# cmusatyalab/mega-nerf

Measured on NVIDIA B200. Metric: ray-samples/sec (MLP+composite), higher is better.
Workload: dtype f16 operands / f32 accumulate

## Files before the change

include/mn_b200.h:

```cpp
#ifndef MN_B200_H
#define MN_B200_H

#include <stddef.h>
#include <stdint.h>

#ifdef __cplusplus
extern "C" {
#endif

#define MN_ABI_VERSION 1

enum {
    MN_OK = 0,
    MN_ERR_INVALID = 1,
    MN_ERR_CUDA = 2,
    MN_ERR_SHAPE = 3,
    MN_ERR_SPHERE = 4,
    MN_ERR_WORKSPACE = 5,
    MN_ERR_UNSUPPORTED = 6
};

enum {
    MN_PREC_FP32 = 0,
    MN_PREC_TC_F16 = 1,
// ... 111 lines not shown


int mn_composite_backward(mn_ctx* ctx, const float* raw_d, const float* z_d, int S, const float* raw2_d,
                          const float* z2_d, int S2, const float* last_delta_d, int64_t N, int flip,
                          const float* grad_rgb_d, const float* grad_lambda_d, float* grad_raw_d, float* grad_raw2_d,
                          void* stream);
int mn_sh_to_rgb_backward(mn_ctx* ctx, int deg, const float* coef_d, int64_t coef_stride, const float* dirs_d,
                          int64_t dir_stride, int dir_div, int64_t B, int apply_sigmoid, const float* grad_out_d,
                          float* grad_coef_d, void* stream);

size_t mn_model_tape_bytes(const mn_model* m, int64_t B);
int mn_model_forward_train(mn_ctx* ctx, mn_model* m, const mn_rows* rows, int64_t B, int use_coarse,
                           const float* sigma_noise_d, float* out_d, void* tape_d, size_t tape_bytes, void* workspace_d,
                           size_t workspace_bytes, void* stream);
#define MN_PARAM_OFFSETS 44
size_t mn_model_backward_workspace_bytes(const mn_model* m, int64_t B);
int64_t mn_model_grad_floats(const mn_model* m);
int mn_model_param_offsets(const mn_model* m, int64_t* out, int n);
int mn_model_backward(mn_ctx* ctx, mn_model* m, int64_t B, int use_coarse, const float* grad_out_d, const void* tape_d,
                      size_t tape_bytes, float* param_grads_d, void* workspace_d, size_t workspace_bytes, void* stream);

int mn_model_train_tc_supported(const mn_model* m);
size_t mn_model_tape_bytes_tc(const mn_model* m, int64_t B);
int mn_model_forward_train_tc(mn_ctx* ctx, mn_model* m, const mn_rows* rows, int64_t B, int use_coarse,
                              const float* sigma_noise_d, float* out_d, void* tape_d, size_t tape_bytes, void* workspace_d,
                              size_t workspace_bytes, void* stream);
size_t mn_model_backward_workspace_bytes_tc(const mn_model* m, int64_t B);
int mn_model_backward_tc(mn_ctx* ctx, mn_model* m, int64_t B, int use_coarse, const float* grad_out_d, const void* tape_d,
                         size_t tape_bytes, float* param_grads_d, void* workspace_d, size_t workspace_bytes, void* stream);

int mn_debug_tp_program(const mn_model_desc* desc, unsigned int* table_out, int cap_entries, int* info8);
int mn_debug_read_trace(unsigned long long* out, unsigned int* counts, int reset);
int mn_debug_read_clock(unsigned long long* out4);

#ifdef __cplusplus
}
#endif
#endif
```

mega_nerf_b200/_cabi.py:

```python
from __future__ import annotations

import ctypes as C
import os
import threading
from typing import Dict, Optional

import torch

_HERE = os.path.dirname(os.path.abspath(__file__))
LIB_PATH = os.path.join(_HERE, 'libmn_b200.so')

MN_OK, MN_ERR_INVALID, MN_ERR_CUDA, MN_ERR_SHAPE, MN_ERR_SPHERE, MN_ERR_WORKSPACE, MN_ERR_UNSUPPORTED = range(7)
PREC_FP32, PREC_TC_F16, PREC_TC_F16X3 = 0, 1, 2
PRECISIONS = {'fp32': PREC_FP32, 'tc_f16': PREC_TC_F16, 'tc_f16x3': PREC_TC_F16X3}

MN_MAX_LAYERS = 16


class ModelDesc(C.Structure):
    _fields_ = [('kind', C.c_int), ('n_sub', C.c_int),
                ('pos_xyz_dim', C.c_int), ('pos_dir_dim', C.c_int), ('layers', C.c_int), ('layer_dim', C.c_int),
                ('appearance_dim', C.c_int), ('affine_appearance', C.c_int), ('appearance_count', C.c_int),
                ('rgb_dim', C.c_int), ('xyz_dim', C.c_int), ('shifted_softplus', C.c_int),
                ('n_skip', C.c_int), ('skip_layers', C.c_int * 8),
                ('boundary_margin', C.c_float), ('xyz_real', C.c_int), ('cluster_dim_start', C.c_int)]


class NerfWeights(C.Structure):
    _fields_ = [('xyz_w', C.c_void_p * MN_MAX_LAYERS), ('xyz_b', C.c_void_p * MN_MAX_LAYERS),
                ('sigma_w', C.c_void_p), ('sigma_b', C.c_void_p), ('final_w', C.c_void_p), ('final_b', C.c_void_p),
                ('dir_a_w', C.c_void_p), ('dir_a_b', C.c_void_p), ('rgb_w', C.c_void_p), ('rgb_b', C.c_void_p),
                ('embedding_a', C.c_void_p), ('affine_w', C.c_void_p), ('affine_b', C.c_void_p)]


class Rows(C.Structure):
    _fields_ = [('mode', C.c_int), ('x_d', C.c_void_p), ('cols', C.c_int), ('dirs_d', C.c_void_p),
                ('dir_stride', C.c_int64), ('idx_d', C.c_void_p), ('samples_per_ray', C.c_int)]


_P, _I, _L, _F, _Z = C.c_void_p, C.c_int, C.c_int64, C.c_float, C.c_size_t
SIGNATURES = {
    'mn_abi_version': (_I, []),
    'mn_create': (_I, [C.POINTER(_P), _I]),
    'mn_destroy': (None, [_P]),
    'mn_last_error': (C.c_char_p, [_P]),
    'mn_check_status': (_I, [_P, _P]),
    'mn_launch_count': (C.c_longlong, [_P]),
    'mn_profile_enable': (_I, [_P, _I]),
    'mn_profile_read': (_I, [_P, C.POINTER(C.c_double), C.POINTER(C.c_longlong)]),
    'mn_ray_directions': (_I, [_P, _I, _I, _F, _F, _F, _F, _I, _P, _P]),
    'mn_rays': (_I, [_P, _P, _I, _P, _I, _L, _F, _F, _I, _F, _F, _P, _P]),
    'mn_rays_pairs': (_I, [_P, _P, _L, _P, _I, _P, _P, _L, _F, _F, _I, _F, _F, _P, _P]),
    'mn_debug_tp_program': (_I, [_P, _P, _I, _P]),
    'mn_debug_read_trace': (_I, [_P, _P, _I]),
    'mn_debug_read_clock': (_I, [_P]),
    'mn_sample_coarse': (_I, [_P, _P, _P, _P, _P, _F, _L, _I, _P, _P, _P]),
    'mn_stratify': (_I, [_P, _P, _L, _P, _F, _L, _I, _P, _P]),
    'mn_points_from_z': (_I, [_P, _P, _P, _L, _I, _P, _P]),
    'mn_sample_pdf': (_I, [_P, _P, _P, _L, _P, _P, _L, _L, _I, _I, _P, _P, _P, _P]),
    'mn_sort_cat': (_I, [_P, _P, _I, _P, _I, _L, _I, _P, _P]),
    'mn_composite': (_I, [_P, _P, _P, _P, _I, _P, _P, _P, _I, _P, _L, _I, _P, _P, _P, _P, _P, _P]),
    'mn_intersect_sphere': (_I, [_P, _P, _P, _P, _L, _P, _P]),
    'mn_points_outside': (_I, [_P, _P, _P, _P, _P, _P, _L, _I, _I, _I, _P, _P, _P]),
    'mn_sh_to_rgb': (_I, [_P, _I, _P, _L, _P, _L, _I, _L, _I, _P, _P]),
    'mn_embed': (_I, [_P, _P, _L, _I, _I, _P, _P]),
    'mn_model_create': (_I, [_P, C.POINTER(ModelDesc), C.POINTER(_P)]),
    'mn_model_destroy': (None, [_P]),
    'mn_model_set_centroids': (_I, [_P, _P, _P]),
    'mn_model_set_weights': (_I, [_P, _I, C.POINTER(NerfWeights), _P]),
    'mn_model_set_max_multiplicity': (_I, [_P, _I]),
    'mn_model_workspace_bytes': (_Z, [_P, _L, _I]),
    'mn_model_forward': (_I, [_P, _P, C.POINTER(Rows), _L, _I, _I, _P, _I, _P, _P, _Z, _P]),
    'mn_model_route': (_I, [_P, _P, C.POINTER(Rows), _L, _P, _P, _P]),
    'mn_model_last_stats': (_I, [_P, _P, C.POINTER(_L), C.POINTER(_L), _P]),
    'mn_render_rays_workspace_bytes': (_Z, [_P, _L, _I, _I, _I, _I, _I]),
    'mn_render_rays': (_I, [_P, _P, _P, _P, _L, _P, _I, _P, _I, _I, _I, _I, _P, _P, _P, _P, _P, _Z, _P]),
    'mn_peer_gather_store': (_I, [_P, _P, _P, _L, _L, C.POINTER(C.c_void_p), _I, _P]),
    'mn_cluster_min_dist_ratios': (_I, [_P, _P, _L, _P, _I, _P, _I, _I, _F, _P, _P, _P]),
    'mn_composite_backward': (_I, [_P, _P, _P, _I, _P, _P, _I, _P, _L, _I, _P, _P, _P, _P, _P]),
    'mn_sh_to_rgb_backward': (_I, [_P, _I, _P, _L, _P, _L, _I, _L, _I, _P, _P, _P]),
    'mn_model_tape_bytes': (_Z, [_P, _L]),
    'mn_model_forward_train': (_I, [_P, _P, C.POINTER(Rows), _L, _I, _P, _P, _P, _Z, _P, _Z, _P]),
    'mn_model_backward_workspace_bytes': (_Z, [_P, _L]),
    'mn_model_grad_floats': (_L, [_P]),
    'mn_model_param_offsets': (_I, [_P, C.POINTER(_L), _I]),
    'mn_model_backward': (_I, [_P, _P, _L, _I, _P, _P, _Z, _P, _P, _Z, _P]),
    'mn_model_train_tc_supported': (_I, [_P]),
    'mn_model_tape_bytes_tc': (_Z, [_P, _L]),
# ... 74 lines not shown
```

mega_nerf_b200/csrc/mn_mlp_tc.cu:

```cuda
#include <cuda_fp16.h>

#include <cstdlib>
#include <cstring>
#include <type_traits>
#include <vector>

#include "mn_model.cuh"

namespace {

constexpr int kTileM = 128;

__device__ unsigned long long g_trace[4 * 4096];
__device__ unsigned int g_trace_n[2];
__device__ __forceinline__ void trace_ev(int on, int who, int ev, int sl, int gi) {
    if (!(on & 1) || blockIdx.x != 0) return;
    const unsigned int i = atomicAdd(&g_trace_n[who], 1u);
    if (i < 2048) {
        unsigned long long t;
        asm volatile("mov.u64 %0, %%globaltimer;" : "=l"(t));
        g_trace[(who * 2048 + i) * 2 + 0] = ((unsigned long long)ev << 32) | ((unsigned long long)sl << 16) | (unsigned long long)gi;
        g_trace[(who * 2048 + i) * 2 + 1] = t;
    }
}
__device__ unsigned long long g_clk[4];
__device__ __forceinline__ void clk_stamp(int on, int which) {
    if (!(on & 1) || blockIdx.x != 0 || threadIdx.x != 0) return;
    unsigned long long t;
    asm volatile("mov.u64 %0, %%globaltimer;" : "=l"(t));
    g_clk[2 * which] = (unsigned long long)clock64();
    g_clk[2 * which + 1] = t;
}
constexpr int kMaxStages = 4;
__host__ __device__ constexpr int ring_slab_cols(bool split) { return split ? 32 : 64; }
__host__ __device__ constexpr int ring_stage_bytes(bool split) { return ring_slab_cols(split) * 256 * 2; }
constexpr int kMaxGemm = 16;
constexpr int kThreads = 576;
constexpr int kEpiWarps = 16;
constexpr int kWarpProd = 16;
constexpr int kWarpMma = 17;
constexpr int kPPThreads = kThreads;

enum { SRC_H = 0, SRC_XPE = 1, SRC_XAUX = 2 };
enum { EPI_RELU = 0, EPI_RELU_SIGMA = 1, EPI_LINEAR = 2, EPI_RGB = 3,
       EPI_D_LINEAR = 4, EPI_D_MASK = 5, EPI_D_MASK_SIGMA = 6 };
enum { PP_INFER = 0, PP_TRAIN_FWD = 1, PP_DGRAD = 2 };

struct TcGemm {
    int n;
    int nseg;
    int src[2];
    int k[2];
    int w_off;
    int bias_off;
    int epi;
};

struct TcPlan {
    int n_gemm, n_trunk;
    TcGemm g[kMaxGemm];
    int kpe, kaux;
    int plane_bytes;
    int f32_floats;
    int sigma_w_off;
// ... 505 lines not shown
        "add.u64 b1, %3, %4;\n\tadd.u64 b2, b1, %4;\n\tadd.u64 b3, b2, %4;\n\t"
        "@e  tcgen05.mma.cta_group::1.kind::f16 [%0], %1, %3, %5, p;\n\t"
        "@q1 tcgen05.mma.cta_group::1.kind::f16 [%0], a1, b1, %5, 1;\n\t"
        "@q2 tcgen05.mma.cta_group::1.kind::f16 [%0], a2, b2, %5, 1;\n\t"
        "@q3 tcgen05.mma.cta_group::1.kind::f16 [%0], a3, b3, %5, 1;\n\t"
        "@e  tcgen05.commit.cta_group::1.mbarrier::arrive::one.shared::cluster.b64 [%8];\n\t}"
        ::"r"(d_tmem), "l"(ad), "l"(a_step), "l"(bd), "l"(b_step), "r"(idesc), "r"(accum), "r"(nk), "r"(empty_bar)
        : "memory");
}


struct TcArgs {
    MlpArgs m;
    TcPlan plan;
    const unsigned char* wpack;
    const __half* ximg;
    int64_t x_plane_halves;
    int split;
    int desc_swap;
    int64_t n_tiles_cap;
    unsigned char* tape_act;
    float* tape_f32;
    unsigned char* tape_dz;
    float* tape_gf32;
    const float* grad_out;
    float* emb_sum;
    const float* scale;
    int64_t act_tile_bytes;
    int layers;
    const unsigned char* tpack;
    size_t tp_sub_bytes;
    const uint4* tp_prog;
    int tp_n[4];
};

struct SmemLayout {
    int ring, h, xa, f32, sigp, bars, total, stages;
};

constexpr int kSmemMax = 227 * 1024;

__host__ __device__ inline SmemLayout smem_layout(const TcPlan& p, bool split) {
    SmemLayout s;
    const int kx = p.kpe > p.kaux ? p.kpe : p.kaux;
    const int fixed = p.L * kTileM * 2 * (split ? 2 : 1) + kx * kTileM * 2 + ((p.f32_floats * 4 + 15) / 16) * 16 + 2048 + 256;
    int st = (kSmemMax - fixed) / ring_stage_bytes(split);
    if (st > kMaxStages) st = kMaxStages;
    s.stages = st;
    s.ring = 0;
    s.h = s.ring + st * ring_stage_bytes(split);
    s.xa = s.h + p.L * kTileM * 2 * (split ? 2 : 1);
    s.f32 = s.xa + kx * kTileM * 2;
    s.sigp = s.f32 + ((p.f32_floats * 4 + 15) / 16) * 16;
    s.bars = s.sigp + 2048;
    s.total = s.bars + 256;
    return s;
}

template <bool kSplit>
__global__ void __launch_bounds__(kThreads, 1) tc_mlp_kernel(const TcArgs A) {
    constexpr int kSlabCols = ring_slab_cols(kSplit);
    constexpr int kStageBytes = ring_stage_bytes(kSplit);
    extern __shared__ __align__(1024) unsigned char smem[];
    const TcPlan& P = A.plan;
    const SmemLayout SL = smem_layout(P, kSplit);
    const int kStages = SL.stages;
// ... 799 lines not shown
    }
    if ((rc = pack(P.g[gi++], Pk + m->lay.rgb_w, nd.rgb_dim, nd.rgb_in, 0, 0, Pk + m->lay.rgb_b, nd.rgb_dim))) return rc;
    mn_pack_push(ctx, PackOp{Pk + m->lay.sigma_w, f32 + P.sigma_w_off, nullptr, (long long)nd.L, PK_TC_F32, {nd.L, 0, 0, 0, 0, 0, 0}});
    mn_pack_push(ctx, PackOp{Pk + m->lay.sigma_b, f32 + P.sigma_w_off + nd.L, nullptr, 4, PK_TC_F32, {1, 0, 0, 0, 0, 0, 0}});
    m->tc_ready = 1;

    TcPlan D;
    m->train_tc_ok = 0;
    if (!wide && build_dgrad_plan(nd, &D)) {
        if (!m->tc_dgrad) {
            MN_CUDA(ctx, cudaMalloc(&m->tc_dgrad, (size_t)D.sub_bytes * m->d.n_sub));
            MN_CUDA(ctx, cudaMemsetAsync(m->tc_dgrad, 0, (size_t)D.sub_bytes * m->d.n_sub, st));
            m->tc_dgrad_sub_bytes = (size_t)D.sub_bytes;
        }
        unsigned char* db = (unsigned char*)m->tc_dgrad + (size_t)sub * D.sub_bytes;
        const float* Q = m->packed_bwd + (size_t)sub * m->blay.total;
        auto packd = [&](const TcGemm& g, const float* wd, int ld) -> int {
            mn_pack_push(ctx, PackOp{wd, db + g.w_off, nullptr, (long long)g.n * g.k[0], PK_DGRAD, {ld, g.n, g.k[0], 0, 0, 0, 0}});
            return MN_OK;
        };
        int di = 0;
        if ((rc = packd(D.g[di++], Q + m->blay.dira_f, nd.L))) return rc;
        if ((rc = packd(D.g[di++], Q + m->blay.final_w, nd.L))) return rc;
        for (int l = nd.layers - 1; l >= 1; --l)
            if ((rc = packd(D.g[di++], Q + m->blay.w[l], nd.L))) return rc;
        float* df32 = reinterpret_cast<float*>(db + D.f32_off);
        mn_pack_push(ctx, PackOp{Pk + m->lay.sigma_w, df32, nullptr, (long long)nd.L, PK_TC_F32, {nd.L, 0, 0, 0, 0, 0, 0}});
        mn_pack_push(ctx, PackOp{Pk + m->lay.rgb_w, df32 + nd.L, nullptr, (long long)3 * (nd.L / 2), PK_RGBW, {nd.L / 2, 3, 0, 0, 0, 0, 0}});
        m->train_tc_ok = 1;
    }
    return MN_OK;
}

int mn_mlp_tc_launch(mn_ctx* ctx, mn_model* m, const MlpArgs& a, int64_t n_tiles128, int precision, void* ws, size_t ws_bytes,
                     cudaStream_t st) {
    TcArgs A{};
    if (!build_plan(a.nd, &A.plan) || !m->tc_ready)
        return mn_fail(ctx, MN_ERR_UNSUPPORTED,
                       "tensor-core MLP path covers layer_dim 64..256 (multiple of 64) or 512 and rgb_dim <= 32; "
                       "use precision 'fp32' for this model");
    if (a.nd.L > 256 && precision == MN_PREC_TC_F16X3)
        return mn_fail(ctx, MN_ERR_UNSUPPORTED,
                       "precision 'tc_f16x3' covers layer_dim <= 256; use 'tc_f16' or 'fp32' for the 512-wide network");
    if (n_tiles128 <= 0) return MN_OK;
    TcPlan& P = A.plan;
    const int split = precision == MN_PREC_TC_F16X3 ? 1 : 0;
    P.sub_bytes = (int)m->tc_sub_bytes;
    A.m = a;
    A.wpack = (const unsigned char*)m->tc_packed;
    A.split = split;
    static int desc_swap = -1;
    if (desc_swap < 0) {
        const char* e = getenv("MN_TC_TRACE");
        desc_swap = e ? atoi(e) : 0;
    }
    A.desc_swap = desc_swap;
    A.n_tiles_cap = n_tiles128;
    const size_t need = mn_mlp_tc_workspace(m, n_tiles128, precision);
    if (ws_bytes < need || !ws) return mn_fail(ctx, MN_ERR_WORKSPACE, "mn_mlp_tc_launch: workspace too small");
    uintptr_t wp = ((uintptr_t)ws + 1023) / 1024 * 1024;
    __half* ximg = reinterpret_cast<__half*>(wp);
    A.ximg = ximg;
    A.x_plane_halves = (int64_t)n_tiles128 * (P.kpe + P.kaux) * kTileM;

    static int use_pp = -1;
    if (use_pp < 0) {
// ... 41 lines not shown
            const unsigned ncl = (unsigned)(groups < ctx->sm_count / 2 ? groups : ctx->sm_count / 2);
            cudaLaunchConfig_t cfg{};
            cfg.gridDim = dim3(2 * ncl);
            cfg.blockDim = dim3(kThreads);
            cfg.dynamicSmemBytes = (size_t)WL.total;
            cfg.stream = st;
            cudaLaunchAttribute at[1];
            at[0].id = cudaLaunchAttributeClusterDimension;
            at[0].val.clusterDim.x = 2;
            at[0].val.clusterDim.y = 1;
            at[0].val.clusterDim.z = 1;
            cfg.attrs = at;
            cfg.numAttrs = 1;
            MN_CUDA(ctx, cudaLaunchKernelEx(&cfg, tc_mlp_wide_kernel<2>, A));
        } else {
            MN_CUDA(ctx, cudaFuncSetAttribute(tc_mlp_wide_kernel<1>, cudaFuncAttributeMaxDynamicSharedMemorySize, WL.total));
            const unsigned grid_w = (unsigned)(n_tiles128 < ctx->sm_count ? n_tiles128 : ctx->sm_count);
            tc_mlp_wide_kernel<1><<<grid_w, kThreads, WL.total, st>>>(A);
        }
        mn_prof_end(ctx, st);
        MN_LAUNCH_CHECK(ctx);
        return MN_OK;
    }
    const SmemLayout SL = smem_layout(P, split != 0);
    const int total = SL.total;
    if (total > kSmemMax || SL.stages < 2) return mn_fail(ctx, MN_ERR_UNSUPPORTED, "tensor-core MLP: shared-memory budget exceeded");
    const unsigned grid = (unsigned)(n_tiles128 < ctx->sm_count ? n_tiles128 : ctx->sm_count);
    if (split) {
        MN_CUDA(ctx, cudaFuncSetAttribute(tc_mlp_kernel<true>, cudaFuncAttributeMaxDynamicSharedMemorySize, total));
        mn_prof_begin(ctx, st);
        tc_mlp_kernel<true><<<grid, kThreads, total, st>>>(A);
    } else {
        if (run_tp) {
            const unsigned grid_tp = (unsigned)((n_tiles128 + 1) / 2 < ctx->sm_count ? (n_tiles128 + 1) / 2 : ctx->sm_count);
            MN_CUDA(ctx, cudaFuncSetAttribute(tc_mlp_tp_kernel, cudaFuncAttributeMaxDynamicSharedMemorySize, TL.total));
            mn_prof_begin(ctx, st);
            tc_mlp_tp_kernel<<<grid_tp, kTPThreads, TL.total, st>>>(A);
        } else if (run_pp) {
            const unsigned grid_pp = (unsigned)((n_tiles128 + 1) / 2 < ctx->sm_count ? (n_tiles128 + 1) / 2 : ctx->sm_count);
            MN_CUDA(ctx, cudaFuncSetAttribute(tc_mlp_pp_kernel<PP_INFER>, cudaFuncAttributeMaxDynamicSharedMemorySize, PL.total));
            mn_prof_begin(ctx, st);
            tc_mlp_pp_kernel<PP_INFER><<<grid_pp, kPPThreads, PL.total, st>>>(A);
        } else {
            MN_CUDA(ctx, cudaFuncSetAttribute(tc_mlp_kernel<false>, cudaFuncAttributeMaxDynamicSharedMemorySize, total));
            mn_prof_begin(ctx, st);
            tc_mlp_kernel<false><<<grid, kThreads, total, st>>>(A);
        }
    }
    mn_prof_end(ctx, st);
    MN_LAUNCH_CHECK(ctx);
    return MN_OK;
}

size_t mn_train_tc_x_tile_bytes(const mn_model* m) {
    TcPlan P;
    return build_plan(m->nd, &P) ? (size_t)P.x_tile_bytes : 0;
}
size_t mn_train_tc_act_tile_bytes(const mn_model* m) {
    const NetDims& nd = m->nd;
    return (size_t)(nd.layers + 1) * nd.L * kTileM * 2 + (size_t)(nd.L / 2) * kTileM * 2;
}

int mn_mlp_tc_launch_train(mn_ctx* ctx, mn_model* m, const MlpArgs& a, int64_t n_tiles128, const TrainTcTape& tape, cudaStream_t st) {
    TcArgs A{};
    if (!m->train_tc_ok || !build_plan(a.nd, &A.plan) || !m->tc_ready)
        return mn_fail(ctx, MN_ERR_UNSUPPORTED, "tensor-core training covers layer_dim 256 with a direction / appearance head and rgb_dim 3; use train precision 'fp32'");
// ... 152 lines not shown
    H.n_tiles = tiles_used;
    H.fixed_sub = a.fixed_sub;
    H.chunk_tiles = 16;
    H.gw = a.gw;
    H.sub_stride = a.lay.total;
    H.sigma_w = a.lay.sigma_w; H.sigma_b = a.lay.sigma_b; H.rgb_w = a.lay.rgb_w; H.rgb_b = a.lay.rgb_b;
    tc_heads_wgrad_kernel<<<dim3((unsigned)mn_cdiv(tiles_used, 16), (unsigned)n_sub), 256, 0, st>>>(H);
    MN_LAUNCH_CHECK(ctx);
    if (nd.app_in_dira) {
        tc_emb_grad_kernel<<<dim3((unsigned)nd.app_count, (unsigned)a.n_sub), 64, 0, st>>>(emb_sum, a.packed_bwd, a.blay.total, a.blay.dira_e, L / 2, nd.app,
                                                                                          nd.app_count, a.gw, a.lay.total, a.lay.emb);
        MN_LAUNCH_CHECK(ctx);
    }
    mn_prof_end(ctx, st);
    return MN_OK;
}

extern "C" int mn_debug_read_clock(unsigned long long* out4) {
    cudaDeviceSynchronize();
    if (out4) cudaMemcpyFromSymbol(out4, g_clk, sizeof(unsigned long long) * 4);
    return 0;
}

extern "C" int mn_debug_read_trace(unsigned long long* out, unsigned int* counts, int reset) {
    cudaDeviceSynchronize();
    if (out) cudaMemcpyFromSymbol(out, g_trace, sizeof(unsigned long long) * 4 * 4096);
    if (counts) cudaMemcpyFromSymbol(counts, g_trace_n, sizeof(unsigned int) * 2);
    if (reset) {
        unsigned int z[2] = {0, 0};
        cudaMemcpyToSymbol(g_trace_n, z, sizeof(z));
    }
    return 0;
}
```

mega_nerf_b200/csrc/mn_mlp_tp.cuh:

```cuda
#pragma once

constexpr int kTPStageBytes = 16384;
constexpr int kTPStageCols = 64;
constexpr int kTPXCols = 16;
constexpr int kTPX0Off = 8192;
constexpr int kTPXBytes = kTPXCols * kTileM * 2;
constexpr int kTPMaxStages = 12;
constexpr int kTPMaxProg = 320;
constexpr int kTPMaxLoads = 160;
constexpr int kTPThreads = kPPThreads + 32;
enum { TF_FIRST = 2, TF_LAST = 4, TF_FROM_X = 8, TF_WAIT_A = 16 };

struct TPLayout {
    int ring, f32, f32_stride, sigp, bars, prog, loads, total, stages;
};

__host__ __device__ inline TPLayout tp_layout(const TcPlan& p) {
    TPLayout s;
    s.f32_stride = ((p.f32_floats * 4 + 15) / 16) * 16;
    const int fixed = s.f32_stride + 2048 + 512 + (kTPMaxProg + kTPMaxLoads) * 16;
    int st = (kSmemMax - fixed) / kTPStageBytes;
    if (st > kTPMaxStages) st = kTPMaxStages;
    s.stages = st;
    s.ring = 0;
    s.f32 = st * kTPStageBytes;
    s.sigp = s.f32 + s.f32_stride;
    s.bars = s.sigp + 2048;
    s.prog = s.bars + 512;
    s.loads = s.prog + kTPMaxProg * 16;
    s.total = s.loads + kTPMaxLoads * 16;
    return s;
}

__host__ __device__ inline int tp_gemm_bytes(const TcGemm& g) {
    const int nw = g.n < 128 ? g.n : 128, nh = (g.n + 127) / 128;
    return (g.k[0] + (g.nseg > 1 ? g.k[1] : 0)) * nw * nh * 2;
}

__device__ __forceinline__ void tp_stage_tmem(uint32_t d_tmem, uint32_t a_tmem, uint64_t bd, uint64_t b_step, uint32_t idesc,
                                              uint32_t accum, uint32_t nk, uint32_t empty_bar, uint32_t release) {
    asm volatile(
        "{\n\t.reg .pred e, p, q1, q2, q3, rl;\n\t.reg .b64 b1, b2, b3;\n\t.reg .b32 a1, a2, a3;\n\t"
        "elect.sync _|e, 0xffffffff;\n\t"
        "setp.ne.b32 p, %5, 0;\n\t"
        "setp.gt.and.u32 q1, %6, 1, e;\n\t"
        "setp.gt.and.u32 q2, %6, 2, e;\n\t"
        "setp.gt.and.u32 q3, %6, 3, e;\n\t"
        "setp.ne.and.b32 rl, %8, 0, e;\n\t"
        "add.u32 a1, %1, 8;\n\tadd.u32 a2, %1, 16;\n\tadd.u32 a3, %1, 24;\n\t"
        "add.u64 b1, %2, %3;\n\tadd.u64 b2, b1, %3;\n\tadd.u64 b3, b2, %3;\n\t"
        "@e  tcgen05.mma.cta_group::1.kind::f16 [%0], [%1], %2, %4, p;\n\t"
        "@q1 tcgen05.mma.cta_group::1.kind::f16 [%0], [a1], b1, %4, 1;\n\t"
        "@q2 tcgen05.mma.cta_group::1.kind::f16 [%0], [a2], b2, %4, 1;\n\t"
        "@q3 tcgen05.mma.cta_group::1.kind::f16 [%0], [a3], b3, %4, 1;\n\t"
        "@rl tcgen05.commit.cta_group::1.mbarrier::arrive::one.shared::cluster.b64 [%7];\n\t}"
        ::"r"(d_tmem), "r"(a_tmem), "l"(bd), "l"(b_step), "r"(idesc), "r"(accum), "r"(nk), "r"(empty_bar), "r"(release)
        : "memory");
}
__device__ __forceinline__ void tp_stage_smem(uint32_t d_tmem, uint64_t ad, uint64_t bd, uint32_t idesc, uint32_t accum,
                                              uint32_t empty_bar, uint32_t release) {
    asm volatile(
        "{\n\t.reg .pred e, p, rl;\n\t"
        "elect.sync _|e, 0xffffffff;\n\t"
        "setp.ne.b32 p, %4, 0;\n\t"
// ... 90 lines not shown
    float sacc = 0.0f;
#pragma unroll
    for (int i = 0; i < 4; ++i) {
        const float4 b = reinterpret_cast<const float4*>(bias16)[i];
        float f0 = __uint_as_float(v[4 * i + 0]) + b.x, f1 = __uint_as_float(v[4 * i + 1]) + b.y;
        float f2 = __uint_as_float(v[4 * i + 2]) + b.z, f3 = __uint_as_float(v[4 * i + 3]) + b.w;
        if (kSigma) {
            f0 = fmaxf(f0, 0.0f); f1 = fmaxf(f1, 0.0f); f2 = fmaxf(f2, 0.0f); f3 = fmaxf(f3, 0.0f);
            const float4 s4 = reinterpret_cast<const float4*>(sw16)[i];
            sacc = fmaf(f0, s4.x, sacc); sacc = fmaf(f1, s4.y, sacc);
            sacc = fmaf(f2, s4.z, sacc); sacc = fmaf(f3, s4.w, sacc);
        }
        uint32_t p0 = pack_h2(f0, f1), p1 = pack_h2(f2, f3);
        if (kRelu && !kSigma) {
            const __half2 z = __float2half2_rn(0.0f);
            __half2 h0 = __hmax2(*reinterpret_cast<__half2*>(&p0), z), h1 = __hmax2(*reinterpret_cast<__half2*>(&p1), z);
            p0 = *reinterpret_cast<const uint32_t*>(&h0);
            p1 = *reinterpret_cast<const uint32_t*>(&h1);
        }
        hp8[2 * i] = p0;
        hp8[2 * i + 1] = p1;
    }
    return sacc;
}

__global__ void __launch_bounds__(kTPThreads, 1) tc_mlp_tp_kernel(const TcArgs A) {
    extern __shared__ __align__(1024) unsigned char smem[];
    const TcPlan& P = A.plan;
    const TPLayout SL = tp_layout(P);
    unsigned char* ring = smem + SL.ring;
    float* F32 = reinterpret_cast<float*>(smem + SL.f32);
    float* SIGP = reinterpret_cast<float*>(smem + SL.sigp);
    uint64_t* bars = reinterpret_cast<uint64_t*>(smem + SL.bars);
    uint64_t* full = bars;
    uint64_t* empty = bars + 12;
    uint64_t* acc_full = bars + 24;
    uint64_t* d_free = bars + 26;
    uint64_t* a_ready = bars + 28;
    uint64_t* f32_full = bars + 30;
    uint64_t* f32_empty = bars + 31;
    uint64_t* turn = bars + 32;
    uint32_t* tmem_slot = reinterpret_cast<uint32_t*>(bars + 34);
    uint4* PROG = reinterpret_cast<uint4*>(smem + SL.prog);
    uint4* LOADS = reinterpret_cast<uint4*>(smem + SL.loads);

    const int warp = threadIdx.x >> 5, lane = threadIdx.x & 31;
    const int64_t n_slots = A.m.counters ? A.m.counters[CNT_NSLOTS] : A.m.B;
    const int64_t n_tiles = (n_slots + kTileM - 1) / kTileM;
    const int n_gemm = A.m.sigma_only ? P.n_trunk : P.n_gemm;
    const int n_prog = A.m.sigma_only ? A.tp_n[1] : A.tp_n[0];
    const int n_loads = A.m.sigma_only ? A.tp_n[3] : A.tp_n[2];
    const float* SW = F32 + P.sigma_w_off;
    const float* RGBB = F32 + P.g[P.n_gemm - 1].bias_off;

    for (int i = threadIdx.x; i < n_prog + 2; i += blockDim.x) PROG[i] = i < n_prog ? A.tp_prog[i] : make_uint4(0u, 0u, 0u, 0u);
    for (int i = threadIdx.x; i < n_loads; i += blockDim.x) LOADS[i] = A.tp_prog[kTPMaxProg + i];
    if (threadIdx.x == 0) {
        for (int i = 0; i < kTPMaxStages; ++i) { mbar_init(&full[i], 1); mbar_init(&empty[i], 2); }
        for (int i = 0; i < 2; ++i) {
            mbar_init(&acc_full[i], 1);
            mbar_init(&d_free[i], kEpiWarps);
            mbar_init(&a_ready[i], kEpiWarps);
        }
        mbar_init(f32_full, 1);
        mbar_init(f32_empty, kEpiWarps);
        mbar_init(&turn[0], 1);
        mbar_init(&turn[1], 1);
        asm volatile("fence.mbarrier_init.release.cluster;" ::: "memory");
    }
    if (warp == kWarpProd) {
        asm volatile("tcgen05.alloc.cta_group::1.sync.aligned.shared::cta.b32 [%0], %1;" ::"r"(smem_u32(tmem_slot)), "n"(512));
        asm volatile("tcgen05.relinquish_alloc_permit.cta_group::1.sync.aligned;");
    }
    tc_fence_before();
    __syncthreads();
    tc_fence_after();
    const uint32_t tmem_base = *tmem_slot;
    clk_stamp(A.desc_swap, 0);

    auto sub_of = [&](int64_t tile) -> int {
        int sub = A.m.fixed_sub;
        if (A.m.counters) {
            sub = 0;
            const int64_t s0 = tile * kTileM;
            while (sub + 1 < A.m.n_sub && s0 >= A.m.counters[CNT_START + sub + 1]) ++sub;
        }
        return sub;
    };
    const int64_t n_pairs = (n_tiles + 1) / 2;
    const uint32_t nst = (uint32_t)SL.stages;

    if (warp == kWarpProd) {
        if (lane == 0) {
            uint32_t stage = 0, phase = 0, fph_e = 0, ahead = 0;
            int last_sub = -1;
            const uint32_t f32_bytes = (uint32_t)SL.f32_stride;
            const uint32_t empty_pa = smem_u32(empty), full_pa = smem_u32(full), ring_pa = smem_u32(ring);
            const int64_t xtile_bytes = (int64_t)(P.kpe + P.kaux) * kTileM * 2;
            for (int64_t pr = blockIdx.x; pr < n_pairs; pr += gridDim.x) {
                const int64_t t0 = 2 * pr;
                const int sub0 = sub_of(t0);
                const unsigned char* wsub = A.tpack + (size_t)sub0 * A.tp_sub_bytes;
                const unsigned char* xt0 = reinterpret_cast<const unsigned char*>(A.ximg) + t0 * xtile_bytes;
                const bool valid1 = t0 + 1 < n_tiles;
                if (sub0 != last_sub) {
                    if (last_sub >= 0) { mbar_wait(f32_empty, fph_e); fph_e ^= 1; }
                    const unsigned char* fsrc = A.wpack + (size_t)sub0 * P.sub_bytes + (size_t)P.f32_off;
                    mbar_expect_tx(f32_full, f32_bytes);
                    bulk_g2s(reinterpret_cast<unsigned char*>(F32), fsrc, f32_bytes, f32_full);
                    last_sub = sub0;
                }
                const uint32_t xbytes = valid1 ? 2u * kTPXBytes : (uint32_t)kTPXBytes;
                for (int e = 0; e < n_loads; ++e) {
                    const uint4 E = LOADS[e];
                    const uint32_t cur = stage;
                    if (!ahead) mbar_wait_a(empty_pa + 8u * cur, phase ^ 1);
                    if (++stage == nst) { stage = 0; phase ^= 1; }
                    ahead = mbar_test_a(empty_pa + 8u * stage, phase ^ 1);
                    const uint32_t bar = full_pa + 8u * cur, dst = ring_pa + cur * (uint32_t)kTPStageBytes;
                    const bool has_x = E.z != 0xFFFFFFFFu;
                    asm volatile("mbarrier.arrive.expect_tx.shared::cta.b64 _, [%0], %1;" ::"r"(bar), "r"(E.y + (has_x ? xbytes : 0u)) : "memory");
                    asm volatile("cp.async.bulk.shared::cluster.global.mbarrier::complete_tx::bytes [%0], [%1], %2, [%3];"
                                 ::"r"(dst), "l"(wsub + E.x), "r"(E.y), "r"(bar) : "memory");
                    if (has_x) {
                        const unsigned char* xs = xt0 + ((int64_t)E.z << 4);
                        asm volatile("cp.async.bulk.shared::cluster.global.mbarrier::complete_tx::bytes [%0], [%1], %2, [%3];"
                                     ::"r"(dst + (uint32_t)kTPX0Off), "l"(xs), "r"((uint32_t)kTPXBytes), "r"(bar) : "memory");
                        if (valid1)
                            asm volatile("cp.async.bulk.shared::cluster.global.mbarrier::complete_tx::bytes [%0], [%1], %2, [%3];"
                                         ::"r"(dst + (uint32_t)(kTPX0Off + kTPXBytes)), "l"(xs + xtile_bytes), "r"((uint32_t)kTPXBytes), "r"(bar)
                                         : "memory");
                    }
                }
            }
        }
    } else if (warp == kWarpMma || warp == kWarpMma + 1) {
        const uint32_t sl = (uint32_t)(warp - kWarpMma);
        uint32_t stage = 0, phase = 0, ahead = 0, dph = 0, aph = 0;
        const uint32_t ring_base = smem_u32(ring);
        const uint32_t full_a = smem_u32(full), empty_a = smem_u32(empty);
        const uint32_t acc_full_a = smem_u32(acc_full) + 8u * sl, d_free_a = smem_u32(d_free) + 8u * sl, a_ready_a = smem_u32(a_ready) + 8u * sl;
        const uint64_t xd = make_desc(ring_base + (uint32_t)kTPX0Off + sl * (uint32_t)kTPXBytes, kTileM * 16, 128);
        const uint64_t bd_base = make_desc(ring_base, 0, 128);
        const uint64_t st_step = (uint64_t)(kTPStageBytes >> 4);
        const uint32_t d_tmem = tmem_base + sl * 256u;
        const uint32_t turn_mine = smem_u32(&turn[sl]), turn_other = smem_u32(&turn[sl ^ 1u]);
        uint32_t tph = sl ? 0u : 1u;
        for (int64_t pr = blockIdx.x; pr < n_pairs; pr += gridDim.x) {
            const bool valid1 = 2 * pr + 1 < n_tiles;
            if (sl && !valid1) break;
            uint4 E = PROG[0];
            for (int e = 0; e < n_prog; ++e) {
                const uint4 En = PROG[e + 1];
                const uint32_t fl = E.z >> 20;
                const uint32_t nw = E.z & 0xFFFu, ns = (E.z >> 12) & 0xFu, nk_last = (E.z >> 16) & 0xFu, idesc = E.y;
                uint32_t a_t = d_tmem + 128u + E.x;
                E = En;
                uint32_t accum = 1;
                if (fl & TF_FIRST) {
                    mbar_wait_a(d_free_a, dph ^ 1);
                    dph ^= 1;
                    accum = 0;
                }
                if (fl & TF_WAIT_A) {
                    mbar_wait_a(a_ready_a, aph);
                    aph ^= 1;
                }
                const uint64_t bdn = bd_base + ((uint64_t)nw << 16);
                const uint64_t b_step = (uint64_t)(2u * nw);
                const uint32_t first = stage;
                if (ns == 4u && nk_last == 4u && !(fl & TF_FROM_X)) {
                    const uint32_t c0 = stage, c1 = c0 + 1 == nst ? 0u : c0 + 1, c2 = c1 + 1 == nst ? 0u : c1 + 1, c3 = c2 + 1 == nst ? 0u : c2 + 1;
                    const uint32_t p0 = phase, p1 = c1 < c0 ? p0 ^ 1u : p0, p2 = c2 < c0 ? p0 ^ 1u : p0, p3 = c3 < c0 ? p0 ^ 1u : p0;
                    if (!ahead) mbar_wait_a(full_a + 8u * c0, p0);
                    mbar_wait_a(full_a + 8u * c1, p1);
                    mbar_wait_a(full_a + 8u * c2, p2);
                    mbar_wait_a(full_a + 8u * c3, p3);
                    const uint32_t nx = c3 + 1 == nst ? 0u : c3 + 1;
                    if (nx < stage) phase ^= 1;
                    stage = nx;
                    ahead = mbar_test_a(full_a + 8u * stage, phase);
// ... 24 lines not shown
                    for (uint32_t s2 = 0; s2 < ns; ++s2) {
                        const uint32_t cur = stage;
                        if (!ahead) mbar_wait_a(full_a + 8u * cur, phase);
                        if (++stage == nst) { stage = 0; phase ^= 1; }
                        ahead = mbar_test_a(full_a + 8u * stage, phase);
                        tc_fence_after();
                        const uint64_t so = (uint64_t)cur * st_step;
                        if (fl & TF_FROM_X) tp_stage_smem(d_tmem, xd + so, bdn + so, idesc, accum, empty_a + 8u * cur, 1u);
                        else {
                            tp_stage_tmem(d_tmem, a_t, bdn + so, b_step, idesc, accum, s2 + 1 == ns ? nk_last : 4u, empty_a + 8u * cur, 1u);
                            a_t += 32u;
                        }
                        accum = 1;
                    }
                }
                if (valid1) {
                    if (lane == 0) asm volatile("mbarrier.arrive.shared::cta.b64 _, [%0];" ::"r"(turn_other) : "memory");
                    __syncwarp();
                } else {
                    uint32_t c = first;
                    for (uint32_t s2 = 0; s2 < ns; ++s2) {
                        commit_elect(empty_a + 8u * c);
                        if (++c == nst) c = 0;
                    }
                }
                if (fl & TF_LAST) commit_elect(acc_full_a);
            }
        }
    } else {
        const int q = warp & 3;
        const int part = warp >> 2;
        const int r = q * 32 + lane;
        const uint32_t t_lane = tmem_base + ((uint32_t)(q * 32) << 16);
        uint32_t aphm = 0, fph0 = 0;
        const uint32_t acc_full_a = smem_u32(acc_full);
        int last_sub = -1;
        const int L = P.L;
        for (int64_t pr = blockIdx.x; pr < n_pairs; pr += gridDim.x) {
            const int64_t t0 = 2 * pr;
            const bool valid1 = t0 + 1 < n_tiles;
            {
                const int sub0 = sub_of(t0);
                if (sub0 != last_sub) {
                    if (last_sub >= 0) {
                        __syncwarp();
                        if (lane == 0) mbar_arrive(f32_empty);
                    }
                    mbar_wait(f32_full, fph0);
                    fph0 ^= 1;
                    last_sub = sub0;
                }
            }
            float sigma_[2] = {0.0f, 0.0f}, sacc_[2] = {0.0f, 0.0f};
            uint32_t keep0[16] = {}, keep1[16] = {};
            for (int gi = 0; gi < n_gemm; ++gi) {
                const int g_n = P.g[gi].n, g_epi = P.g[gi].epi;
                const int nh = (g_n + 127) >> 7;
                const float* bias = F32 + P.g[gi].bias_off;
                const bool want_sigma = g_epi == EPI_RELU_SIGMA;
                const bool publish = g_epi != EPI_RGB && !(want_sigma && A.m.sigma_only);
                if (g_epi == EPI_RGB) {
                    for (int sl = 0; sl < (valid1 ? 2 : 1); ++sl) {
                        mbar_wait(&acc_full[sl], (aphm >> sl) & 1u);
                        aphm ^= 1u << sl;
                        tc_fence_after();
                        const int64_t slot = (t0 + sl) * kTileM + r;
                        const int64_t row = slot < n_slots ? (A.m.slot_row ? (int64_t)A.m.slot_row[slot] : slot) : -1;
                        uint32_t v[32];
                        tmem_ld32(t_lane + (uint32_t)sl * 256u, v);
                        tmem_ld_wait();
                        tc_fence_before();
                        __syncwarp();
                        if (lane == 0) mbar_arrive(&d_free[sl]);
                        if (part == 0 && row >= 0)
                            tc_emit_rgb(A.m, A.m.nd.affine ? sub_of(t0 + sl) : 0, row, slot, v, RGBB, sl ? sigma_[1] : sigma_[0], nullptr);
                    }
                    continue;
                }
                for (int h = 0; h < nh; ++h) {
                    const int n0 = 128 * h + 32 * part;
                    const bool active = n0 < g_n;
                    const bool last_h = h == nh - 1;
                    const int nb = active ? n0 : 0;
                    const float* b16 = bias + nb;
                    const float* s16 = SW + nb;
                    const uint32_t c_src = (uint32_t)(active ? 32 * part : 0);
                    const bool stash_out = publish && nh == 2;
                    auto do_slot = [&](auto slc, auto reluc, auto sigc, auto lastc, uint32_t (&keep)[16]) {
                        constexpr int sl = decltype(slc)::value;
                        constexpr bool kRelu = decltype(reluc)::value, kSigma = decltype(sigc)::value, kLast = decltype(lastc)::value;
                        mbar_wait_a(acc_full_a + 8u * sl, (aphm >> sl) & 1u);
// ... 39 lines not shown
                                    float sv = ((SIGP[r] + SIGP[kTileM + r]) + (SIGP[2 * kTileM + r] + SIGP[3 * kTileM + r])) + SW[L];
                                    if (A.m.sigma_noise && row >= 0) sv = sv + A.m.sigma_noise[row];
                                    const float sg = A.m.nd.softplus ? mn_softplus_shifted(sv) : fmaxf(sv, 0.0f);
                                    sigma_[sl] = sg;
                                    if (A.m.sigma_only && row >= 0) {
                                        const int64_t o = (A.m.scatter ? row : slot) * A.m.out_cols;
                                        A.m.out[o] = A.m.slot_w ? sg * A.m.slot_w[slot] : sg;
                                    }
                                }
                                asm volatile("bar.sync 1, 512;" ::: "memory");
                            }
                        } else {
                            float sacc = tp_piece16<kRelu, kSigma>(v0, b16, s16, keep);
                            sacc += tp_piece16<kRelu, kSigma>(v1, b16 + 16, s16 + 16, keep + 8);
                            if (kSigma) sacc_[sl] += sacc;
                        }
                    };
                    using T = std::true_type;
                    using F = std::false_type;
                    using S0 = std::integral_constant<int, 0>;
                    using S1 = std::integral_constant<int, 1>;
                    if (g_epi == EPI_RELU) {
                        if (last_h) { do_slot(S0{}, T{}, F{}, T{}, keep0); if (valid1) do_slot(S1{}, T{}, F{}, T{}, keep1); }
                        else        { do_slot(S0{}, T{}, F{}, F{}, keep0); if (valid1) do_slot(S1{}, T{}, F{}, F{}, keep1); }
                    } else if (g_epi == EPI_LINEAR) {
                        if (last_h) { do_slot(S0{}, F{}, F{}, T{}, keep0); if (valid1) do_slot(S1{}, F{}, F{}, T{}, keep1); }
                        else        { do_slot(S0{}, F{}, F{}, F{}, keep0); if (valid1) do_slot(S1{}, F{}, F{}, F{}, keep1); }
                    } else {
                        if (last_h) { do_slot(S0{}, T{}, T{}, T{}, keep0); if (valid1) do_slot(S1{}, T{}, T{}, T{}, keep1); }
                        else        { do_slot(S0{}, T{}, T{}, F{}, keep0); if (valid1) do_slot(S1{}, T{}, T{}, F{}, keep1); }
                    }
                }
            }
        }
    }
    tc_fence_before();
    __syncthreads();
    clk_stamp(A.desc_swap, 1);
    if (warp == kWarpProd) {
        asm volatile("tcgen05.dealloc.cta_group::1.sync.aligned.b32 %0, %1;" ::"r"(tmem_base), "n"(512));
    }
}

static bool tp_build_program(const TcPlan& P, std::vector<uint4>* table, int counts[4]) {
    std::vector<uint4> prog, loads;
    int woff = 0;
    counts[1] = counts[3] = -1;
    for (int gi = 0; gi < P.n_gemm; ++gi) {
        if (gi == P.n_trunk) { counts[1] = (int)prog.size(); counts[3] = (int)loads.size(); }
        const TcGemm& g = P.g[gi];
        const int nw = g.n < 128 ? g.n : 128, nh = (g.n + 127) / 128;
        const int K = g.k[0] + (g.nseg > 1 ? g.k[1] : 0);
        for (int h = 0; h < nh; ++h) {
            const int himg = woff + h * K * nw * 2;
            int kbase = 0;
            bool waited = false;
            for (int sgi = 0; sgi < g.nseg; ++sgi) {
                const bool fx = g.src[sgi] != SRC_H;
                const int step = fx ? kTPXCols : kTPStageCols;
                const int kk = g.k[sgi];
                const int ns = (kk + step - 1) / step;
                if (ns > kTPMaxStages - 4) return false;
                for (int j = 0; j < ns; ++j) {
                    const int k0 = j * step, kc = kk - k0 < step ? kk - k0 : step;
                    const unsigned xo = fx ? (unsigned)(((g.src[sgi] == SRC_XAUX ? P.kpe * kTileM * 2 : 0) + k0 * kTileM * 2) >> 4) : 0xFFFFFFFFu;
                    loads.push_back(make_uint4((unsigned)(himg + (kbase + k0) * nw * 2), (unsigned)(kc * nw * 2), xo, 0u));
// ... 25 lines not shown
```

Measured before the change: 593.5 million.

## Double-buffer per-submodule f32 params and use contiguous pair ranges per CTA

The f32 bias/sigma parameter area in shared memory is now double-buffered, so the producer can prefetch the next submodule's f32 block while the epilogue still reads the current one, instead of stalling on a single-buffer empty barrier. Pair scheduling changes from a grid-strided loop to contiguous blocks per CTA, which reduces submodule switches per CTA. A debug pair-timing trace is also added, gated on a desc_swap bit. The second f32 buffer costs shared memory, which may reduce pipeline stages, and contiguous ranges can cause load imbalance at the tail.

```diff
diff --git a/include/mn_b200.h b/include/mn_b200.h
--- a/include/mn_b200.h
+++ b/include/mn_b200.h
@@ -167,6 +167,7 @@
 int mn_debug_tp_program(const mn_model_desc* desc, unsigned int* table_out, int cap_entries, int* info8);
 int mn_debug_read_trace(unsigned long long* out, unsigned int* counts, int reset);
 int mn_debug_read_clock(unsigned long long* out4);
+int mn_debug_read_pair_trace(unsigned long long* out, long long cap_records, int reset);
 
 #ifdef __cplusplus
 }
diff --git a/mega_nerf_b200/_cabi.py b/mega_nerf_b200/_cabi.py
--- a/mega_nerf_b200/_cabi.py
+++ b/mega_nerf_b200/_cabi.py
@@ -54,6 +54,7 @@
     'mn_debug_tp_program': (_I, [_P, _P, _I, _P]),
     'mn_debug_read_trace': (_I, [_P, _P, _I]),
     'mn_debug_read_clock': (_I, [_P]),
+    'mn_debug_read_pair_trace': (_I, [_P, C.c_longlong, _I]),
     'mn_sample_coarse': (_I, [_P, _P, _P, _P, _P, _F, _L, _I, _P, _P, _P]),
     'mn_stratify': (_I, [_P, _P, _L, _P, _F, _L, _I, _P, _P]),
     'mn_points_from_z': (_I, [_P, _P, _P, _L, _I, _P, _P]),
diff --git a/mega_nerf_b200/csrc/mn_mlp_tc.cu b/mega_nerf_b200/csrc/mn_mlp_tc.cu
--- a/mega_nerf_b200/csrc/mn_mlp_tc.cu
+++ b/mega_nerf_b200/csrc/mn_mlp_tc.cu
@@ -30,6 +30,11 @@
     asm volatile("mov.u64 %0, %%globaltimer;" : "=l"(t));
     g_clk[2 * which] = (unsigned long long)clock64();
     g_clk[2 * which + 1] = t;
+}
+__device__ __forceinline__ unsigned long long gtimer() {
+    unsigned long long t;
+    asm volatile("mov.u64 %0, %%globaltimer;" : "=l"(t));
+    return t;
 }
 constexpr int kMaxStages = 4;
 __host__ __device__ constexpr int ring_slab_cols(bool split) { return split ? 32 : 64; }
@@ -601,6 +606,9 @@
     size_t tp_sub_bytes;
     const uint4* tp_prog;
     int tp_n[4];
+    unsigned long long* pair_trace;
+    int64_t pair_trace_base;
+    unsigned int pair_trace_launch;
 };
 
 struct SmemLayout {
@@ -1466,6 +1474,24 @@
     return MN_OK;
 }
 
+constexpr int64_t kTPTraceCap = 1 << 17;
+static unsigned long long* g_pair_trace_d = nullptr;
+static int64_t g_pair_trace_used = 0;
+static unsigned int g_pair_trace_launches = 0;
+
+static void tp_trace_reserve(TcArgs* A, int64_t pairs_cap) {
+    if (!g_pair_trace_d) {
+        const size_t bytes = sizeof(unsigned long long) * kTPTraceWords * kTPTraceCap;
+        if (cudaMalloc(&g_pair_trace_d, bytes) != cudaSuccess) { g_pair_trace_d = nullptr; return; }
+        cudaMemset(g_pair_trace_d, 0, bytes);
+    }
+    if (g_pair_trace_used + pairs_cap > kTPTraceCap) return;
+    A->pair_trace = g_pair_trace_d;
+    A->pair_trace_base = g_pair_trace_used;
+    A->pair_trace_launch = g_pair_trace_launches++;
+    g_pair_trace_used += pairs_cap;
+}
+
 int mn_mlp_tc_launch(mn_ctx* ctx, mn_model* m, const MlpArgs& a, int64_t n_tiles128, int precision, void* ws, size_t ws_bytes,
                      cudaStream_t st) {
     TcArgs A{};
@@ -1573,6 +1599,7 @@
         tc_mlp_kernel<true><<<grid, kThreads, total, st>>>(A);
     } else {
         if (run_tp) {
+            if (desc_swap & 1) tp_trace_reserve(&A, (n_tiles128 + 1) / 2);
             const unsigned grid_tp = (unsigned)((n_tiles128 + 1) / 2 < ctx->sm_count ? (n_tiles128 + 1) / 2 : ctx->sm_count);
             MN_CUDA(ctx, cudaFuncSetAttribute(tc_mlp_tp_kernel, cudaFuncAttributeMaxDynamicSharedMemorySize, TL.total));
             mn_prof_begin(ctx, st);
@@ -1791,3 +1818,17 @@
     }
     return 0;
 }
+
+extern "C" int mn_debug_read_pair_trace(unsigned long long* out, long long cap_records, int reset) {
+    cudaDeviceSynchronize();
+    const int64_t n = g_pair_trace_used;
+    if (out && g_pair_trace_d && cap_records > 0)
+        cudaMemcpy(out, g_pair_trace_d, sizeof(unsigned long long) * kTPTraceWords * (size_t)(n < cap_records ? n : cap_records),
+                   cudaMemcpyDeviceToHost);
+    if (reset) {
+        if (g_pair_trace_d) cudaMemset(g_pair_trace_d, 0, sizeof(unsigned long long) * kTPTraceWords * kTPTraceCap);
+        g_pair_trace_used = 0;
+        g_pair_trace_launches = 0;
+    }
+    return (int)n;
+}
diff --git a/mega_nerf_b200/csrc/mn_mlp_tp.cuh b/mega_nerf_b200/csrc/mn_mlp_tp.cuh
--- a/mega_nerf_b200/csrc/mn_mlp_tp.cuh
+++ b/mega_nerf_b200/csrc/mn_mlp_tp.cuh
@@ -10,26 +10,46 @@
 constexpr int kTPMaxLoads = 160;
 constexpr int kTPThreads = kPPThreads + 32;
 enum { TF_FIRST = 2, TF_LAST = 4, TF_FROM_X = 8, TF_WAIT_A = 16 };
+constexpr int kTPTraceWords = 6;
+
+enum {
+    TPB_FULL = 0,
+    TPB_EMPTY = TPB_FULL + kTPMaxStages,
+    TPB_ACC_FULL = TPB_EMPTY + kTPMaxStages,
+    TPB_D_FREE = TPB_ACC_FULL + 2,
+    TPB_A_READY = TPB_D_FREE + 2,
+    TPB_F32_FULL = TPB_A_READY + 2,
+    TPB_F32_EMPTY = TPB_F32_FULL + 2,
+    TPB_TURN = TPB_F32_EMPTY + 2,
+    TPB_TMEM_SLOT = TPB_TURN + 2,
+    TPB_COUNT
+};
 
 struct TPLayout {
     int ring, f32, f32_stride, sigp, bars, prog, loads, total, stages;
 };
 
 __host__ __device__ inline TPLayout tp_layout(const TcPlan& p) {
+    static_assert(TPB_COUNT * 8 <= 512, "mbarriers exceed the layout's barrier area");
     TPLayout s;
     s.f32_stride = ((p.f32_floats * 4 + 15) / 16) * 16;
-    const int fixed = s.f32_stride + 2048 + 512 + (kTPMaxProg + kTPMaxLoads) * 16;
+    const int fixed = 2 * s.f32_stride + 2048 + 512 + (kTPMaxProg + kTPMaxLoads) * 16;
     int st = (kSmemMax - fixed) / kTPStageBytes;
     if (st > kTPMaxStages) st = kTPMaxStages;
     s.stages = st;
     s.ring = 0;
     s.f32 = st * kTPStageBytes;
-    s.sigp = s.f32 + s.f32_stride;
+    s.sigp = s.f32 + 2 * s.f32_stride;
     s.bars = s.sigp + 2048;
     s.prog = s.bars + 512;
     s.loads = s.prog + kTPMaxProg * 16;
     s.total = s.loads + kTPMaxLoads * 16;
     return s;
+}
+
+__host__ __device__ inline void tp_pair_range(int64_t n_pairs, int64_t b, int64_t G, int64_t* lo, int64_t* hi) {
+    *lo = b * n_pairs / G;
+    *hi = (b + 1) * n_pairs / G;
 }
 
 __host__ __device__ inline int tp_gemm_bytes(const TcGemm& g) {
@@ -186,15 +206,15 @@
     float* F32 = reinterpret_cast<float*>(smem + SL.f32);
     float* SIGP = reinterpret_cast<float*>(smem + SL.sigp);
     uint64_t* bars = reinterpret_cast<uint64_t*>(smem + SL.bars);
-    uint64_t* full = bars;
-    uint64_t* empty = bars + 12;
-    uint64_t* acc_full = bars + 24;
-    uint64_t* d_free = bars + 26;
-    uint64_t* a_ready = bars + 28;
-    uint64_t* f32_full = bars + 30;
-    uint64_t* f32_empty = bars + 31;
-    uint64_t* turn = bars + 32;
-    uint32_t* tmem_slot = reinterpret_cast<uint32_t*>(bars + 34);
+    uint64_t* full = bars + TPB_FULL;
+    uint64_t* empty = bars + TPB_EMPTY;
+    uint64_t* acc_full = bars + TPB_ACC_FULL;
+    uint64_t* d_free = bars + TPB_D_FREE;
+    uint64_t* a_ready = bars + TPB_A_READY;
+    uint64_t* f32_full = bars + TPB_F32_FULL;
+    uint64_t* f32_empty = bars + TPB_F32_EMPTY;
+    uint64_t* turn = bars + TPB_TURN;
+    uint32_t* tmem_slot = reinterpret_cast<uint32_t*>(bars + TPB_TMEM_SLOT);
     uint4* PROG = reinterpret_cast<uint4*>(smem + SL.prog);
     uint4* LOADS = reinterpret_cast<uint4*>(smem + SL.loads);
 
@@ -204,8 +224,7 @@
     const int n_gemm = A.m.sigma_only ? P.n_trunk : P.n_gemm;
     const int n_prog = A.m.sigma_only ? A.tp_n[1] : A.tp_n[0];
     const int n_loads = A.m.sigma_only ? A.tp_n[3] : A.tp_n[2];
-    const float* SW = F32 + P.sigma_w_off;
-    const float* RGBB = F32 + P.g[P.n_gemm - 1].bias_off;
+    const int f32_floats = SL.f32_stride / 4;
 
     for (int i = threadIdx.x; i < n_prog + 2; i += blockDim.x) PROG[i] = i < n_prog ? A.tp_prog[i] : make_uint4(0u, 0u, 0u, 0u);
     for (int i = threadIdx.x; i < n_loads; i += blockDim.x) LOADS[i] = A.tp_prog[kTPMaxProg + i];
@@ -216,8 +235,10 @@
             mbar_init(&d_free[i], kEpiWarps);
             mbar_init(&a_ready[i], kEpiWarps);
         }
-        mbar_init(f32_full, 1);
-        mbar_init(f32_empty, kEpiWarps);
+        for (int i = 0; i < 2; ++i) {
+            mbar_init(&f32_full[i], 1);
+            mbar_init(&f32_empty[i], kEpiWarps);
+        }
         mbar_init(&turn[0], 1);
         mbar_init(&turn[1], 1);
         asm volatile("fence.mbarrier_init.release.cluster;" ::: "memory");
@@ -242,26 +263,42 @@
         return sub;
     };
     const int64_t n_pairs = (n_tiles + 1) / 2;
+    int64_t pr_lo, pr_hi;
+    tp_pair_range(n_pairs, blockIdx.x, gridDim.x, &pr_lo, &pr_hi);
     const uint32_t nst = (uint32_t)SL.stages;
 
     if (warp == kWarpProd) {
         if (lane == 0) {
-            uint32_t stage = 0, phase = 0, fph_e = 0, ahead = 0;
+            uint32_t stage = 0, phase = 0, ahead = 0;
+            uint32_t fb = 1, f32_used = 0, fph_e = 0;
             int last_sub = -1;
             const uint32_t f32_bytes = (uint32_t)SL.f32_stride;
             const uint32_t empty_pa = smem_u32(empty), full_pa = smem_u32(full), ring_pa = smem_u32(ring);
             const int64_t xtile_bytes = (int64_t)(P.kpe + P.kaux) * kTileM * 2;
-            for (int64_t pr = blockIdx.x; pr < n_pairs; pr += gridDim.x) {
+            for (int64_t pr = pr_lo; pr < pr_hi; ++pr) {
                 const int64_t t0 = 2 * pr;
                 const int sub0 = sub_of(t0);
                 const unsigned char* wsub = A.tpack + (size_t)sub0 * A.tp_sub_bytes;
                 const unsigned char* xt0 = reinterpret_cast<const unsigned char*>(A.ximg) + t0 * xtile_bytes;
                 const bool valid1 = t0 + 1 < n_tiles;
+                unsigned long long* rec = A.pair_trace ? A.pair_trace + (A.pair_trace_base + pr) * kTPTraceWords : nullptr;
+                if (rec) {
+                    rec[0] = ((unsigned long long)A.pair_trace_launch << 40) | ((unsigned long long)blockIdx.x << 20) | (unsigned)sub0;
+                    rec[1] = (unsigned long long)pr | ((unsigned long long)n_pairs << 32);
+                    rec[2] = gtimer();
+                }
                 if (sub0 != last_sub) {
-                    if (last_sub >= 0) { mbar_wait(f32_empty, fph_e); fph_e ^= 1; }
+                    fb ^= 1;
+                    if (f32_used & (1u << fb)) {
+                        if (rec) rec[3] = gtimer();
+                        mbar_wait(&f32_empty[fb], (fph_e >> fb) & 1u);
+                        fph_e ^= 1u << fb;
+                        if (rec) rec[4] = gtimer();
+                    }
+                    f32_used |= 1u << fb;
                     const unsigned char* fsrc = A.wpack + (size_t)sub0 * P.sub_bytes + (size_t)P.f32_off;
-                    mbar_expect_tx(f32_full, f32_bytes);
-                    bulk_g2s(reinterpret_cast<unsigned char*>(F32), fsrc, f32_bytes, f32_full);
+                    mbar_expect_tx(&f32_full[fb], f32_bytes);
+                    bulk_g2s(reinterpret_cast<unsigned char*>(F32 + fb * f32_floats), fsrc, f32_bytes, &f32_full[fb]);
                     last_sub = sub0;
                 }
                 const uint32_t xbytes = valid1 ? 2u * kTPXBytes : (uint32_t)kTPXBytes;
@@ -300,7 +337,7 @@
         const uint32_t d_tmem = tmem_base + sl * 256u;
         const uint32_t turn_mine = smem_u32(&turn[sl]), turn_other = smem_u32(&turn[sl ^ 1u]);
         uint32_t tph = sl ? 0u : 1u;
-        for (int64_t pr = blockIdx.x; pr < n_pairs; pr += gridDim.x) {
+        for (int64_t pr = pr_lo; pr < pr_hi; ++pr) {
             const bool valid1 = 2 * pr + 1 < n_tiles;
             if (sl && !valid1) break;
             uint4 E = PROG[0];
@@ -391,11 +428,13 @@
         const int part = warp >> 2;
         const int r = q * 32 + lane;
         const uint32_t t_lane = tmem_base + ((uint32_t)(q * 32) << 16);
-        uint32_t aphm = 0, fph0 = 0;
+        uint32_t aphm = 0, fph = 0;
         const uint32_t acc_full_a = smem_u32(acc_full);
         int last_sub = -1;
+        uint32_t eb = 1;
+        const float* F32e = F32;
         const int L = P.L;
-        for (int64_t pr = blockIdx.x; pr < n_pairs; pr += gridDim.x) {
+        for (int64_t pr = pr_lo; pr < pr_hi; ++pr) {
             const int64_t t0 = 2 * pr;
             const bool valid1 = t0 + 1 < n_tiles;
             {
@@ -403,19 +442,23 @@
                 if (sub0 != last_sub) {
                     if (last_sub >= 0) {
                         __syncwarp();
-                        if (lane == 0) mbar_arrive(f32_empty);
+                        if (lane == 0) mbar_arrive(&f32_empty[eb]);
                     }
-                    mbar_wait(f32_full, fph0);
-                    fph0 ^= 1;
+                    eb ^= 1;
+                    mbar_wait(&f32_full[eb], (fph >> eb) & 1u);
+                    fph ^= 1u << eb;
+                    F32e = F32 + eb * f32_floats;
                     last_sub = sub0;
                 }
             }
+            const float* SW = F32e + P.sigma_w_off;
+            const float* RGBB = F32e + P.g[P.n_gemm - 1].bias_off;
             float sigma_[2] = {0.0f, 0.0f}, sacc_[2] = {0.0f, 0.0f};
             uint32_t keep0[16] = {}, keep1[16] = {};
             for (int gi = 0; gi < n_gemm; ++gi) {
                 const int g_n = P.g[gi].n, g_epi = P.g[gi].epi;
                 const int nh = (g_n + 127) >> 7;
-                const float* bias = F32 + P.g[gi].bias_off;
+                const float* bias = F32e + P.g[gi].bias_off;
                 const bool want_sigma = g_epi == EPI_RELU_SIGMA;
                 const bool publish = g_epi != EPI_RGB && !(want_sigma && A.m.sigma_only);
                 if (g_epi == EPI_RGB) {
@@ -521,6 +564,7 @@
                     }
                 }
             }
+            if (A.pair_trace && warp == 0 && lane == 0) A.pair_trace[(A.pair_trace_base + pr) * kTPTraceWords + 5] = gtimer();
         }
     }
     tc_fence_before();
```

Result: faster. 610.3 million (median of 6 runs) (+2.8%).
